# albertz/ParseOggVorbis

Hardware: AMD Instinct MI355X
Metric: audio packets/sec (blocksize 2048, stereo) (higher is better)
Workload: dtype f32; 1 GPU; config3: 65536 stereo packets, blocksize 2048, 64 streams x 1024, floor+coupling+IMDCT+window+overlap-add; packets_per_gpu=65536, parallelism=streams sharded over 1 GPU(s), no data-path collective

## Files before the change

### parseoggvorbis_amd/csrc/vorbis_synth_hip.hip

```cpp
#include <hip/hip_runtime.h>

#include <math.h>
#include <stdarg.h>
#include <stdio.h>
#include <string.h>

#include <algorithm>
#include <cmath>
#include <mutex>
#include <numeric>
#include <string>
#include <vector>

#include <stdlib.h>

#include "vsyn_device.h"
#include "vsyn_staged.h"
#include "vsyn_prep.h"
#include "vsyn_fused.h"
#include "vsyn_fused_u.h"
#include "vsyn_vq.h"
#include "vsyn_pcm.h"
#include "vsyn_features.h"
#include "vsyn_spectral.h"
// ... 224 lines not shown

static int build_const(const vsyn_setup* su, uint32_t max_streams, vsyn_handle* h, const char** err) {
  if (!su) return fail(err, VSYN_ERR_INVALID, "setup is NULL");
  if (su->channels < 1 || su->channels > VSYN_MAX_CHANNELS) return fail(err, VSYN_ERR_INVALID, "channels %u not in 1..%d", su->channels, VSYN_MAX_CHANNELS);
  if (!is_pow2(su->blocksize0) || !is_pow2(su->blocksize1) || su->blocksize0 < VSYN_MIN_BLOCKSIZE ||
      su->blocksize1 > VSYN_MAX_BLOCKSIZE || su->blocksize0 > su->blocksize1)
    return fail(err, VSYN_ERR_INVALID, "blocksizes %u/%u invalid (hpp:1294-1298)", su->blocksize0, su->blocksize1);
  if (su->num_floors < 1 || su->num_floors > VSYN_MAX_TABLES || su->num_mappings < 1 || su->num_mappings > VSYN_MAX_TABLES ||
      su->num_modes < 1 || su->num_modes > VSYN_MAX_TABLES || !su->floors || !su->mappings || !su->modes)
    return fail(err, VSYN_ERR_INVALID, "floor/mapping/mode counts out of range");
  if (max_streams < 1) return fail(err, VSYN_ERR_INVALID, "max_streams must be >= 1");

  ConstHeader& H = h->H;
  memset(&H, 0, sizeof(H));
  H.channels = su->channels;
  H.bs[0] = su->blocksize0;
  H.bs[1] = su->blocksize1;
  H.lg[0] = ilog2(su->blocksize0);
  H.lg[1] = ilog2(su->blocksize1);
  H.num_floors = su->num_floors;
  H.num_mappings = su->num_mappings;
  H.num_modes = su->num_modes;
  H.max_streams = max_streams;

  std::vector<FloorConst> floors(su->num_floors);
  uint32_t maxp = 2;
  for (uint32_t f = 0; f < su->num_floors; ++f) {
    const vsyn_floor1& sf = su->floors[f];
    FloorConst& fc = floors[f];
    memset(&fc, 0, sizeof(fc));
    if (sf.multiplier < 1 || sf.multiplier > 4) return fail(err, VSYN_ERR_INVALID, "floor %u: multiplier %u (hpp:486-492)", f, sf.multiplier);
    if (sf.num_posts < 2 || sf.num_posts > VSYN_MAX_POSTS || !sf.xs) return fail(err, VSYN_ERR_INVALID, "floor %u: %u posts", f, sf.num_posts);
    static const uint32_t range_of[5] = {0, 256, 128, 86, 64};
    fc.mult = sf.multiplier;
    fc.posts = sf.num_posts;
    fc.range = range_of[sf.multiplier];
    maxp = std::max(maxp, sf.num_posts);
    for (uint32_t i = 0; i < sf.num_posts; ++i) {
      if (sf.xs[i] > 0xFFFFu) return fail(err, VSYN_ERR_INVALID, "floor %u: x[%u]=%u too large", f, i, sf.xs[i]);
      fc.xs[i] = (uint16_t)sf.xs[i];
    }
    if (sf.xs[0] != 0) return fail(err, VSYN_ERR_INVALID, "floor %u: xs[0] must be 0 (hpp:449)", f);
    std::vector<uint32_t> order(sf.num_posts);
    for (uint32_t i = 0; i < sf.num_posts; ++i) order[i] = i;
    std::stable_sort(order.begin(), order.end(), [&](uint32_t a, uint32_t b) { return sf.xs[a] < sf.xs[b]; });
    for (uint32_t s = 0; s < sf.num_posts; ++s) {
      if (s && sf.xs[order[s]] == sf.xs[order[s - 1]]) return fail(err, VSYN_ERR_INVALID, "floor %u: duplicate x %u (render_line needs x0<x1, Utils.hpp:145)", f, sf.xs[order[s]]);
      fc.sorted_idx[s] = (uint8_t)order[s];
      fc.xs_sorted[s] = (uint16_t)sf.xs[order[s]];
    }
    for (uint32_t i = 2; i < sf.num_posts; ++i) {
      int lo = -1, hi = -1;
      for (uint32_t j = 0; j < i; ++j) {
        if (sf.xs[j] < sf.xs[i] && (lo < 0 || sf.xs[j] > sf.xs[lo])) lo = (int)j;
        if (sf.xs[j] > sf.xs[i] && (hi < 0 || sf.xs[j] < sf.xs[hi])) hi = (int)j;
      }
      if (lo < 0 || hi < 0) return fail(err, VSYN_ERR_INVALID, "floor %u: post %u has no low/high neighbour (xs[1] must be the maximum)", f, i);
      fc.lo[i] = (uint8_t)lo;
      fc.hi[i] = (uint8_t)hi;
      fc.pk[i].lo = (uint16_t)lo;
      fc.pk[i].hi = (uint16_t)hi;
      fc.pk[i].dxi = (uint16_t)(sf.xs[i] - sf.xs[lo]);
      fc.pk[i].adx = (uint16_t)(sf.xs[hi] - sf.xs[lo]);
      fc.pk[i].inv_adx = 1.0f / (float)(sf.xs[hi] - sf.xs[lo]);
      fc.pk[i].idx = i;
    }
    {
      std::vector<uint32_t> depth(sf.num_posts, 0);
      uint32_t maxd = 0;
      for (uint32_t i = 2; i < sf.num_posts; ++i) {
        depth[i] = 1u + std::max(depth[fc.lo[i]], depth[fc.hi[i]]);
        maxd = std::max(maxd, depth[i]);
      }
      uint32_t ng = 0;
      for (uint32_t d = 1; d <= maxd; ++d) {
        std::vector<uint32_t> at;
        for (uint32_t i = 2; i < sf.num_posts; ++i)
          if (depth[i] == d) at.push_back(i);
        for (size_t k = 0; k < at.size(); k += 4, ++ng)
          for (uint32_t e = 0; e < 4; ++e) fc.sched[ng][e] = fc.pk[at[std::min(k + e, at.size() - 1)]];
      }
      fc.ngroups = ng;
    }
    if (sf.num_posts <= 32)
      for (uint32_t i = 2; i < sf.num_posts; ++i) fc.pk[i].idx = (1u << fc.lo[i]) | (1u << fc.hi[i]) | (1u << i);
  }
  H.ys_stride = (maxp + 3u) & ~3u;
  h->prep_lds_bytes = maxp > 32 ? H.ys_stride * PREP_THREADS * (uint32_t)sizeof(uint32_t) : 16u;
  h->unwrap_lds_bytes = maxp > 32 ? H.ys_stride * UNWRAP_THREADS * (uint32_t)sizeof(uint32_t) : 16u;

  std::vector<MapConst> maps(su->num_mappings);
  for (uint32_t m = 0; m < su->num_mappings; ++m) {
    const vsyn_mapping& sm = su->mappings[m];
    MapConst& mc = maps[m];
    memset(&mc, 0, sizeof(mc));
    if (sm.num_couplings > 256 || (sm.num_couplings && !sm.couplings) || !sm.channel_floor) return fail(err, VSYN_ERR_INVALID, "mapping %u invalid", m);
    mc.ncoup = sm.num_couplings;
    for (uint32_t k = 0; k < sm.num_couplings; ++k) {
      const vsyn_coupling& c = sm.couplings[k];
      if (c.magnitude == c.angle || c.magnitude >= su->channels || c.angle >= su->channels)
        return fail(err, VSYN_ERR_INVALID, "mapping %u coupling %u invalid (hpp:788-790)", m, k);
      mc.coup[2 * k] = c.magnitude;
      mc.coup[2 * k + 1] = c.angle;
    }
    for (uint32_t c = 0; c < su->channels; ++c) {
      if (sm.channel_floor[c] >= su->num_floors) return fail(err, VSYN_ERR_INVALID, "mapping %u: floor index out of range (hpp:807)", m);
      mc.chfloor[c] = sm.channel_floor[c];
    }
  }
  for (uint32_t k = 0; k < su->num_modes; ++k) {
    if (su->modes[k].mapping >= su->num_mappings) return fail(err, VSYN_ERR_INVALID, "mode %u: mapping out of range (hpp:832)", k);
    H.mode_blockflag[k] = su->modes[k].block_flag ? 1 : 0;
    H.mode_mapping[k] = su->modes[k].mapping;
  }

  size_t off = align_up(sizeof(ConstHeader), 256);
  H.off_floor = (uint32_t)off;
  off = align_up(off + sizeof(FloorConst) * floors.size(), 256);
  H.off_map = (uint32_t)off;
  off = align_up(off + sizeof(MapConst) * maps.size(), 256);
  H.off_invdb = (uint32_t)off;
  off = align_up(off + 256 * sizeof(float), 256);
  for (int b = 0; b < 2; ++b) {
    const uint32_t n = H.bs[b];
    H.off_pre[b] = (uint32_t)off;
    off = align_up(off + (n / 4) * sizeof(float2), 256);
    H.off_post[b] = (uint32_t)off;
    off = align_up(off + (n / 4) * sizeof(float2), 256);
    H.off_fft[b] = (uint32_t)off;
    off = align_up(off + (n / 4) * sizeof(float2), 256);
    H.off_win[b] = (uint32_t)off;
    off = align_up(off + 4 * (size_t)n * sizeof(float), 256);
  }
  H.total_bytes = (uint32_t)off;
  h->host_const.assign(off, 0);
  uint8_t* base = h->host_const.data();
  memcpy(base, &H, sizeof(H));
  memcpy(base + H.off_floor, floors.data(), sizeof(FloorConst) * floors.size());
  memcpy(base + H.off_map, maps.data(), sizeof(MapConst) * maps.size());
  memcpy(base + H.off_invdb, k_inverse_db_bits, sizeof(k_inverse_db_bits));
  for (int b = 0; b < 2; ++b) {
    const uint32_t n = H.bs[b], M = n / 2, N4 = n / 4;
    float2* pre = (float2*)(base + H.off_pre[b]);
    float2* post = (float2*)(base + H.off_post[b]);
    float2* tw = (float2*)(base + H.off_fft[b]);
    for (uint32_t k = 0; k < N4; ++k) {
      const double a = -M_PI * (4.0 * k + 1.0) / (4.0 * M);
      pre[k] = make_float2((float)cos(a), (float)sin(a));
      const double p = -M_PI * (double)k / (double)M;
      post[k] = make_float2((float)cos(p), (float)sin(p));
      const double t = -2.0 * M_PI * (double)k / (double)N4;
      tw[k] = make_float2((float)cos(t), (float)sin(t));
    }
    float* win = (float*)(base + H.off_win[b]);
    for (int w = 0; w < 4; ++w) host_window(H.bs[0], H.bs[1], b, w & 1, (w >> 1) & 1, win + (size_t)w * n);
  }
  return VSYN_OK;
}

extern "C" {

const char* vsyn_version(void) { return "parseoggvorbis_amd vsyn 0.1 (gfx950)"; }
int vsyn_abi_version(void) { return VSYN_ABI_VERSION; }

int vsyn_create(const vsyn_setup* setup, int device, uint32_t max_streams, vsyn_handle** out, const char** err) {
  if (!out) return fail(err, VSYN_ERR_INVALID, "out is NULL");
  *out = nullptr;
  int ndev = 0;
// ... 1733 lines not shown
```

### parseoggvorbis_amd/csrc/vsyn_device.h

```cpp
#pragma once
#include <stdint.h>

#include "../../include/vorbis_synth_hip.h"

#define VSYN_SCHED_GROUPS 64
#define VSYN_MAX_TABLES 64

struct FloorConst {
  uint32_t mult, posts, range;
  uint16_t xs[VSYN_MAX_POSTS + 1];
  uint16_t xs_sorted[VSYN_MAX_POSTS + 1];
  uint8_t sorted_idx[VSYN_MAX_POSTS + 3];
  uint8_t lo[VSYN_MAX_POSTS + 3];
  uint8_t hi[VSYN_MAX_POSTS + 3];
  struct PostK {
    uint16_t lo, hi;
    uint16_t dxi, adx;
    float inv_adx;
    uint32_t idx;
  } pk[VSYN_MAX_POSTS + 1];
  uint32_t ngroups, pad_[3];
  PostK sched[VSYN_SCHED_GROUPS][4];
};

struct MapConst {
  uint32_t ncoup;
  uint8_t chfloor[VSYN_MAX_CHANNELS];
  uint16_t coup[2 * 256];
};

struct ConstHeader {
  uint32_t channels, bs[2], lg[2], ys_stride, num_floors, num_mappings, num_modes, max_streams;
  uint32_t off_floor, off_map, off_invdb;
  uint32_t off_pre[2], off_post[2], off_fft[2], off_win[2];
  uint8_t mode_blockflag[VSYN_MAX_TABLES], mode_mapping[VSYN_MAX_TABLES];
  uint32_t total_bytes;
};

struct PktInfo {
  uint64_t res_off;
  uint32_t out_pos;
  uint32_t emit;
  uint32_t used;
  uint32_t own;
  uint16_t n;
  uint8_t lng, widx;
  uint8_t mapping, bad;
  uint16_t pad;
};

struct SegInfo {
  uint32_t has_carry;
  uint32_t carry_n;
  uint32_t parity_in;
  uint32_t total_emit;
};

struct StreamState {
  uint64_t abs_total_pos;
  uint32_t has_prev, prev_n, parity;
  uint32_t tag;
  uint32_t prev_tail;
};

struct DevStatus {
  uint32_t flags, first_bad_packet;
};

#ifdef __HIPCC__
#define VSYN_CPOL_NT 2
typedef float vsyn_nt_f2 __attribute__((ext_vector_type(2)));
typedef float vsyn_nt_f4 __attribute__((ext_vector_type(4)));
__device__ __forceinline__ float2 stream_load2(const float2* p) {
  const vsyn_nt_f2 v = __builtin_nontemporal_load((const vsyn_nt_f2*)p);
  return make_float2(v.x, v.y);
}
__device__ __forceinline__ void stream_store2(float* p, float a, float b) { __builtin_nontemporal_store(vsyn_nt_f2{a, b}, (vsyn_nt_f2*)p); }
__device__ __forceinline__ void stream_store4(float* p, float a, float b, float c, float d) {
  __builtin_nontemporal_store(vsyn_nt_f4{a, b, c, d}, (vsyn_nt_f4*)p);
}
#endif
#ifdef __HIPCC__
__device__ __forceinline__ const ConstHeader* hdr_of(const uint8_t* cb) { return (const ConstHeader*)cb; }
__device__ __forceinline__ const FloorConst* floor_of(const uint8_t* cb, uint32_t f) {
  return (const FloorConst*)(cb + hdr_of(cb)->off_floor) + f;
}
__device__ __forceinline__ const MapConst* map_of(const uint8_t* cb, uint32_t m) {
  return (const MapConst*)(cb + hdr_of(cb)->off_map) + m;
}
__device__ __forceinline__ const float* invdb_of(const uint8_t* cb) { return (const float*)(cb + hdr_of(cb)->off_invdb); }
__device__ __forceinline__ const float2* pre_of(const uint8_t* cb, int b) { return (const float2*)(cb + hdr_of(cb)->off_pre[b]); }
__device__ __forceinline__ const float2* post_of(const uint8_t* cb, int b) { return (const float2*)(cb + hdr_of(cb)->off_post[b]); }
__device__ __forceinline__ const float2* fft_of(const uint8_t* cb, int b) { return (const float2*)(cb + hdr_of(cb)->off_fft[b]); }
__device__ __forceinline__ const float* win_of(const uint8_t* cb, int b, int widx) {
  return (const float*)(cb + hdr_of(cb)->off_win[b]) + (size_t)widx * hdr_of(cb)->bs[b];
}

__device__ __forceinline__ void raise_status(DevStatus* st, uint32_t flag, uint32_t pkt) {
  atomicOr(&st->flags, flag);
  atomicMin(&st->first_bad_packet, pkt);
}

__device__ __forceinline__ StreamState state_read(const StreamState* __restrict__ st, uint32_t stream, uint32_t epoch, uint32_t* slot) {
  const StreamState a = st[2u * stream], b = st[2u * stream + 1u];
  const uint32_t da = (a.tag == 0u || a.tag == epoch) ? 0xFFFFFFFFu : epoch - a.tag;
// ... 43 lines not shown
```

### parseoggvorbis_amd/csrc/vsyn_floor1.h

```cpp
#pragma once
#include <hip/hip_runtime.h>

#include "vsyn_device.h"

typedef __attribute__((address_space(3))) uint32_t floor1_lds_u32;

__device__ __forceinline__ uint32_t render_point_u32(uint32_t x0, uint32_t y0, uint32_t x1, uint32_t y1, uint32_t X) {
  uint32_t adx = x1 - x0;
  bool up = y1 >= y0;
  uint32_t ady = up ? y1 - y0 : y0 - y1;
  uint32_t off = (ady * (X - x0)) / adx;
  return up ? y0 + off : y0 - off;
}

__device__ __forceinline__ void floor1_unwrap_rows(const uint8_t* cb, const uint16_t* ys, uint16_t* fy, DevStatus* status, const bool act,
                                                   const uint32_t fl_id, const uint32_t p, const size_t gid, const uint32_t stride,
                                                   floor1_lds_u32* const col, const uint32_t NT) {
  const FloorConst* const floors = (const FloorConst*)(cb + hdr_of(cb)->off_floor);
  typedef uint32_t u32x16 __attribute__((ext_vector_type(16)));
  typedef const __attribute__((address_space(4))) u32x16* const_grp;
  typedef const __attribute__((address_space(4))) uint32_t* kptr;
  uint64_t todo = __ballot(act);
  while (todo) {
    const uint32_t f = __builtin_amdgcn_readlane(fl_id, (uint32_t)__builtin_ctzll(todo));
    const bool mine = act && fl_id == f;
    todo &= ~__ballot(mine);
    const FloorConst* fc = floors + f;
    const uint32_t posts = *(kptr)(uintptr_t)&fc->posts, range = *(kptr)(uintptr_t)&fc->range, mult = *(kptr)(uintptr_t)&fc->mult;
    const uint32_t ngroups = *(kptr)(uintptr_t)&fc->ngroups;
    if (!mine) continue;
    if (posts <= 32u) {
      uint32_t fr[32];
      const uint2* in8 = (const uint2*)(ys + gid * stride);
      uint2 win[8];
#pragma unroll
      for (uint32_t j = 0; j < 8; ++j) {
        win[j] = make_uint2(0u, 0u);
        if (j * 4 < posts) win[j] = in8[j];
      }
      uint32_t flags = 3;
      bool bad = false;
      typedef const __attribute__((address_space(4))) u32x16* const_pk4;
      for (int attempt = 0; attempt < 2; ++attempt) {
        const bool exact = attempt == 1;
#pragma unroll
        for (uint32_t j = 0; j < 8; ++j) {
          fr[4 * j + 0] = win[j].x & 0xFFFFu;
          fr[4 * j + 1] = win[j].x >> 16;
          fr[4 * j + 2] = win[j].y & 0xFFFFu;
          fr[4 * j + 3] = win[j].y >> 16;
        }
        flags = 3;
        bad = false;
        uint32_t big_acc = 0;
        auto step = [&](const uint32_t i, const uint32_t kx, const uint32_t ky, const uint32_t kz, const uint32_t touched) {
          const uint32_t lo = kx & 0xFFFFu, hi = kx >> 16;
          const uint32_t val = fr[i], ylo = fr[lo], yhi = fr[hi];
          const uint32_t dxi = ky & 0xFFFFu, adx = ky >> 16;
          const bool up = yhi >= ylo;
          const uint32_t ady = up ? yhi - ylo : ylo - yhi;
          const uint32_t prod = ady * dxi;
          uint32_t off;
          if (exact) {
            off = prod / adx;
          } else {
            off = (uint32_t)(((float)prod + 0.5f) * __uint_as_float(kz));
            big_acc |= prod >> 21;
          }
          const uint32_t predicted = up ? ylo + off : ylo - off;
          const bool ok = predicted <= range;
          const uint32_t pr = ok ? predicted : 0u;
          const uint32_t high_room = range - pr;
          const uint32_t m = min(high_room, pr);
          const uint32_t d = val - m;
          const uint32_t dbig = high_room > pr ? d : ~d;
          const uint32_t dsmall = (val >> 1) ^ (0u - (val & 1u));
          const uint32_t delta = val >= 2u * m ? dbig : dsmall;
          const uint32_t fn = val == 0 ? pr : pr + delta;
          flags |= val != 0 ? touched : 0u;
          bad = bad || !ok;
          fr[i] = bad ? 0u : fn;
        };
        u32x16 kn = *(const_pk4)(uintptr_t)&fc->pk[2];
        for (uint32_t i = 2; i < posts; i += 4) {
          const u32x16 kq = kn;
          kn = *(const_pk4)(uintptr_t)&fc->pk[i + 4];
          step(i, kq[0], kq[1], kq[2], kq[3]);
          if (i + 1 < posts) step(i + 1, kq[4], kq[5], kq[6], kq[7]);
          if (i + 2 < posts) step(i + 2, kq[8], kq[9], kq[10], kq[11]);
          if (i + 3 < posts) step(i + 3, kq[12], kq[13], kq[14], kq[15]);
        }
        if (exact || !__any(big_acc != 0u)) break;
        if (big_acc == 0u) break;
      }
      uint2* out8 = (uint2*)(fy + gid * stride);
      if (bad) raise_status(status, VSYN_ST_FLOOR_RANGE, p);
#pragma unroll
      for (uint32_t j = 0; j < 8; ++j) {
        if (j * 4 >= posts) break;
        uint32_t w[4];
#pragma unroll
        for (uint32_t e = 0; e < 4; ++e) {
          const uint32_t i = 4 * j + e;
          uint32_t v = fr[i] * mult;
          if (v > 0x7FFFu || fr[i] > 0x7FFFu) v = 0x7FFFu;
          w[e] = i < posts ? (bad ? 0x8000u : (v | (((flags >> i) & 1u) << 15))) : 0u;
        }
        out8[j] = make_uint2(w[0] | (w[1] << 16), w[2] | (w[3] << 16));
      }
      continue;
    }
    {
      const uint2* in8 = (const uint2*)(ys + gid * stride);
      for (uint32_t j = 0; j * 4 < posts; ++j) {
        const uint2 w = in8[j];
        col[(4 * j + 0) * NT] = w.x & 0xFFFFu;
        col[(4 * j + 1) * NT] = w.x >> 16;
        col[(4 * j + 2) * NT] = w.y & 0xFFFFu;
        col[(4 * j + 3) * NT] = w.y >> 16;
      }
    }
    uint64_t flags_lo = 3;
    uint32_t flag_64 = 0;
    bool bad = false;
    u32x16 kn = *(const_grp)(uintptr_t)&fc->sched[0][0];
    for (uint32_t gi = 0; gi < ngroups; ++gi) {
      const u32x16 kq = kn;
      kn = *(const_grp)(uintptr_t)&fc->sched[gi + 1u < VSYN_SCHED_GROUPS ? gi + 1u : gi][0];
      uint32_t val[4], ylo[4], yhi[4], fn[4], prod[4], off[4];
#pragma unroll
      for (int e = 0; e < 4; ++e) {
        val[e] = col[kq[4 * e + 3] * NT];
        ylo[e] = col[(kq[4 * e] & 0xFFFFu) * NT];
        yhi[e] = col[(kq[4 * e] >> 16) * NT];
      }
      bool any_big = false;
#pragma unroll
      for (int e = 0; e < 4; ++e) {
        const uint32_t dxi = kq[4 * e + 1] & 0xFFFFu;
        const bool up = yhi[e] >= ylo[e];
        const uint32_t ady = up ? yhi[e] - ylo[e] : ylo[e] - yhi[e];
        prod[e] = ady * dxi;
        off[e] = (uint32_t)(((float)prod[e] + 0.5f) * __uint_as_float(kq[4 * e + 2]));
        any_big = any_big || prod[e] >= (1u << 21) || ady >= 65536u;
      }
      if (__any(any_big)) {
#pragma unroll
        for (int e = 0; e < 4; ++e) {
          const bool up = yhi[e] >= ylo[e];
          const uint32_t ady = up ? yhi[e] - ylo[e] : ylo[e] - yhi[e];
          if (prod[e] >= (1u << 21) || ady >= 65536u) off[e] = prod[e] / (kq[4 * e + 1] >> 16);
        }
      }
#pragma unroll
      for (int e = 0; e < 4; ++e) {
        const bool up = yhi[e] >= ylo[e];
        const uint32_t predicted = up ? ylo[e] + off[e] : ylo[e] - off[e];
        const bool ok = predicted <= range;
        const uint32_t pr = ok ? predicted : 0u;
        const uint32_t high_room = range - pr, low_room = pr;
        const uint32_t room = min(high_room, low_room) * 2;
        const uint32_t big = high_room > low_room ? val[e] - low_room + pr : pr - val[e] + high_room - 1;
        const uint32_t small = (val[e] & 1u) ? pr - (val[e] + 1) / 2 : pr + val[e] / 2;
        fn[e] = val[e] == 0 ? pr : (val[e] >= room ? big : small);
        const uint32_t lo = kq[4 * e] & 0xFFFFu, hi = kq[4 * e] >> 16, i = kq[4 * e + 3];
        const uint64_t touched = (1ull << lo) | (1ull << hi) | (i < 64u ? 1ull << i : 0ull);
        flags_lo |= val[e] != 0 ? touched : 0ull;
        flag_64 |= (val[e] != 0 && i >= 64u) ? 1u : 0u;
        bad = bad || !ok;
      }
#pragma unroll
      for (int e = 0; e < 4; ++e) col[kq[4 * e + 3] * NT] = bad ? 0u : fn[e];
    }
    uint2* out8 = (uint2*)(fy + gid * stride);
    if (bad) raise_status(status, VSYN_ST_FLOOR_RANGE, p);
    for (uint32_t j = 0; j * 4 < posts; ++j) {
      uint32_t w[4];
#pragma unroll
      for (uint32_t e = 0; e < 4; ++e) {
        const uint32_t i = 4 * j + e;
        const uint32_t fv = i < posts ? col[i * NT] : 0u;
        uint32_t v = fv * mult;
        if (v > 0x7FFFu || fv > 0x7FFFu) v = 0x7FFFu;
        const uint32_t fl = i < 64 ? (uint32_t)((flags_lo >> i) & 1ull) : (i == 64 ? flag_64 : 0u);
        w[e] = i < posts ? (bad ? 0x8000u : (v | (fl << 15))) : 0u;
      }
      out8[j] = make_uint2(w[0] | (w[1] << 16), w[2] | (w[3] << 16));
    }
  }
}

// ... 13 lines not shown
```

### parseoggvorbis_amd/csrc/vsyn_prep.h

```cpp
#pragma once
#include <hip/hip_runtime.h>

#include "vsyn_device.h"
#include "vsyn_floor1.h"
#include "vsyn_staged.h"

#define PREP_MAX_SEG_PACKETS 4096u
#define PREP_WAVES 4
#define PREP_THREADS (PREP_WAVES * 64)

struct PrepCtx {
  const uint8_t* cb;
  const vsyn_packet* packets;
  const vsyn_segment* segs;
  const uint16_t* ys;
  uint16_t* fy;
  PktInfo* info;
  SegInfo* sinfo;
  StreamState* state;
  DevStatus* status;
  uint32_t* emit_len;
  uint8_t* run_cls;
  uint64_t plane_stride, long_modes;
  uint32_t S, R, runs_per_seg, fused_ok, P, epoch;
// ... 49 lines not shown
    const uint64_t r = s_res[w];
    if (w < wv) {
      pre = abs_combine(pre, a);
      rpre += r;
    }
    tot = abs_combine(tot, a);
    rtot += r;
  }
  inc = abs_combine(pre, inc);
  rinc += rpre;
  *total = tot;
  *rtotal = rtot;
}

__global__ void __launch_bounds__(PREP_THREADS) vsyn_prep_kernel(const PrepCtx A) {
  extern __shared__ __attribute__((aligned(16))) uint32_t s_rows[];
  __shared__ AbsScan s_abs[PREP_WAVES];
  __shared__ uint64_t s_res[PREP_WAVES];
  __shared__ uint32_t s_pk[PREP_THREADS];
  __shared__ uint32_t s_longbits[PREP_MAX_SEG_PACKETS / 32 + 2];
  __shared__ uint32_t s_last_n;
  const uint8_t* __restrict__ cb = A.cb;
  const ConstHeader* H = hdr_of(cb);
  const uint32_t t = threadIdx.x, lane = t & 63u, wave = __builtin_amdgcn_readfirstlane(t >> 6);
  const uint32_t NT = blockDim.x;
  const uint32_t C = H->channels;
  const uint32_t xj = blockIdx.x >> 3;
  const uint32_t role = (xj ^ (xj >> 5)) & 1u, bid = ((xj >> 1) << 3) | (blockIdx.x & 7u);
  const uint32_t g = bid / A.chunks_per_seg, ch = bid % A.chunks_per_seg;
  if (g >= A.S) return;
#ifdef PREP_STAMPS
  unsigned long long pst_acc[PREP_NSTAMPS] = {0, 0, 0, 0, 0, 0, 0, 0};
  unsigned long long pst_last = __builtin_readcyclecounter();
  const unsigned long long pst_t0 = __builtin_amdgcn_s_memrealtime();
#define PSTAMP_FLUSH()                                                                                              \
  do {                                                                                                              \
    const uint32_t unit_ = blockIdx.x * PREP_WAVES + wave;                                                          \
    if (lane == 0 && unit_ < 8192) {                                                                                \
      for (int i_ = 0; i_ < 5; ++i_) g_prep_stamps[unit_][i_] = pst_acc[i_];                                        \
      g_prep_stamps[unit_][5] = pst_t0;                                                                             \
      g_prep_stamps[unit_][6] = __builtin_amdgcn_s_memrealtime();                                                   \
      g_prep_stamps[unit_][7] = 1ull + role;                                                                        \
    }                                                                                                               \
  } while (0)
#else
#define PSTAMP_FLUSH() do { } while (0)
#endif
  const vsyn_segment sg = A.segs[g];
  const uint32_t num = sg.num_packets;
  const uint32_t R = A.R;
  const uint32_t run0 = ch * A.chunk_runs;
  const uint32_t run1 = min(A.runs_per_seg, run0 + A.chunk_runs);
  const uint32_t cs = run0 * R;
  uint8_t* const cls_row = A.run_cls + (size_t)g * A.runs_per_seg;
  if (sg.stream >= H->max_streams || (uint64_t)sg.first_packet + sg.num_packets > A.P || (sg.residue_off & 3)) {
    if (role) return;
    for (uint32_t r = run0 + t; r < run1; r += NT) cls_row[r] = 0xFFu;
    if (ch == 0u && t == 0u) {
      raise_status(A.status, VSYN_ST_BAD_SEGMENT, sg.first_packet < A.P ? sg.first_packet : 0);
      A.sinfo[g] = SegInfo{0, 0, 0, 0};
    }
    return;
  }
  const uint32_t ce = min(num, run1 * R);
  const vsyn_packet* const spk = A.packets + sg.first_packet;
  typedef uint32_t u32x4 __attribute__((ext_vector_type(4)));
  const uint32_t num_modes = H->num_modes, bs0 = H->bs[0], bs1 = H->bs[1];
  const uint64_t long_modes = A.long_modes;
#define PREP_IS_LONG(m) ((m) < num_modes && (m) < 64u && ((long_modes >> (m)) & 1ull))
#define PREP_N_OF_MODE(m) (PREP_IS_LONG(m) ? bs1 : bs0)
  if (role) {
    const uint32_t ce = min(num, run1 * R);
    if (cs >= ce) return;
    const vsyn_packet* const spk = A.packets + sg.first_packet;
    const uint32_t stride = __builtin_amdgcn_readfirstlane(H->ys_stride);
    const MapConst* const maps = (const MapConst*)(cb + H->off_map);
    const uint32_t chan_mask = C >= 32 ? 0xFFFFFFFFu : ((1u << C) - 1u);
    const uint32_t num_modes = H->num_modes;
    const uint32_t ppp = NT / C;
    for (uint32_t base = cs; base < ce; base += ppp) {
      const uint32_t pe = min(ce, base + ppp);
      const uint32_t rp = t / C, c = t - rp * C;
      const bool row_ok = rp < pe - base;
      uint32_t kmode = 0xFFFFFFFFu, fused_mask = 0;
      if (row_ok) {
        typedef uint32_t u32x2 __attribute__((ext_vector_type(2)));
        const u32x2 w = *(const u32x2*)(spk + base + rp);
        kmode = w.x & 0xFFu;
        fused_mask = w.y;
      }
      const bool mode_ok = row_ok && kmode < num_modes;
      uint32_t fl_id = 0xFFFFFFFFu;
      {
        typedef const __attribute__((address_space(4))) uint32_t* kptr;
        uint64_t todo = __ballot(mode_ok);
        while (todo) {
          const uint32_t m = __builtin_amdgcn_readlane(kmode, (uint32_t)__builtin_ctzll(todo));
          const bool mine = mode_ok && kmode == m;
          todo &= ~__ballot(mine);
          const uint32_t mw = *(kptr)(uintptr_t)((const uint8_t*)H->mode_mapping + (m & ~3u));
          const uint32_t mp = (mw >> (8u * (m & 3u))) & 0xFFu;
          if (mine) fl_id = maps[mp].chfloor[c];
        }
      }
      const bool act = mode_ok && (((fused_mask & chan_mask) >> c) & 1u);
      const uint32_t prow = sg.first_packet + base + rp;
      PSTAMP(3);
      floor1_unwrap_rows(A.cb, A.ys, A.fy, A.status, act, fl_id, prow, (size_t)prow * C + c, stride, (floor1_lds_u32*)s_rows + t, NT);
      PSTAMP(4);
    }
    PSTAMP_FLUSH();
    return;
  }
  uint32_t st_slot;
  const StreamState st0 = state_read(A.state, sg.stream, A.epoch, &st_slot);
  const bool reset = (sg.flags & VSYN_SEG_RESET) != 0;
  const uint32_t carry_n = (!reset && st0.has_prev) ? st0.prev_n : 0;
  const int64_t abs0 = reset ? 0 : (int64_t)st0.abs_total_pos;
  SegInfo si;
  si.has_carry = carry_n ? 1u : 0u;
  si.carry_n = carry_n;
  si.parity_in = reset ? 0u : st0.parity;
  si.total_emit = 0;
  if (cs >= num) {
    for (uint32_t r = run0 + t; r < run1; r += NT) cls_row[r] = 0xFFu;
    if (num == 0u && ch == 0u && t == 0u) {
      A.sinfo[g] = si;
      if (reset) state_write(A.state, sg.stream, st_slot, StreamState{0, 0, 0, 0, 0}, A.epoch);
    }
    return;
  }
  PSTAMP(0);

  AbsScan cin = {0, 0};
  uint64_t cres = 0;
  uint32_t prev_n_in = carry_n;
  uint32_t prev_tail_in = carry_n ? st0.prev_tail : 0u;
  bool halo_long = !carry_n;
  if (cs > 0u) {
    const uint32_t per = (cs + NT - 1u) / NT;
    const uint32_t b = min(cs, t * per), e = min(cs, b + per);
    AbsScan agg = {0, 0};
    uint64_t res = 0;
    uint32_t prev_n = 0;
    if (b < e) prev_n = b == 0u ? carry_n : PREP_N_OF_MODE((uint32_t)spk[b - 1u].mode);
    constexpr uint32_t KEEP = 8;
    for (uint32_t base = b; base < e; base += KEEP) {
      u32x4 kq[KEEP];
#pragma unroll
      for (uint32_t j = 0; j < KEEP; ++j)
        if (base + j < e) kq[j] = *(const u32x4*)(spk + base + j);
#pragma unroll
      for (uint32_t j = 0; j < KEEP; ++j)
        if (base + j < e) {
          const uint32_t md = kq[j].x & 0xFFu;
          const uint32_t n = PREP_N_OF_MODE(md);
          const int64_t gran = (int64_t)((uint64_t)kq[j].z | ((uint64_t)kq[j].w << 32));
          agg = abs_combine(agg, abs_element(gran, prev_n ? (int64_t)(prev_n / 4 + n / 4) : 0));
          res += (uint64_t)C * (n / 2);
          prev_n = n;
        }
    }
    prep_block_scan(agg, res, s_abs, s_res, &cin, &cres);
    const uint32_t hm = __builtin_amdgcn_readfirstlane((uint32_t)spk[cs - 1u].mode);
    prev_n_in = PREP_N_OF_MODE(hm);
    halo_long = PREP_IS_LONG(hm);
    prev_tail_in = prev_tail_of(PREP_IS_LONG(hm), (uint8_t)__builtin_amdgcn_readfirstlane((uint32_t)spk[cs - 1u].next_long));
  }
  PSTAMP(1);

  const uint32_t stride = __builtin_amdgcn_readfirstlane(H->ys_stride);
  const MapConst* const maps = (const MapConst*)(cb + H->off_map);
  const uint32_t chan_mask = C >= 32 ? 0xFFFFFFFFu : ((1u << C) - 1u);
  const uint32_t ppp = NT / C;
  for (uint32_t w = t; w < (ce - cs + 1u + 31u) / 32u; w += NT) s_longbits[w] = 0u;
  __syncthreads();
  if (t == 0u && halo_long) s_longbits[0] = 1u;
  for (uint32_t base = cs; base < ce; base += ppp) {
    const uint32_t pe = min(ce, base + ppp);
    const uint32_t q = base + t;
    const bool valid = q < pe;
    vsyn_packet k = {};
    if (valid) {
      const u32x4 w = *(const u32x4*)(spk + q);
      k.mode = (uint8_t)(w.x & 0xFFu);
      k.prev_long = (uint8_t)((w.x >> 8) & 0xFFu);
      k.next_long = (uint8_t)((w.x >> 16) & 0xFFu);
      k.floor_used = w.y;
      k.granule = (int64_t)((uint64_t)w.z | ((uint64_t)w.w << 32));
    }
    const bool mode_ok = valid && k.mode < num_modes;
// ... 116 lines not shown
```

### parseoggvorbis_amd/csrc/vsyn_staged.h

```cpp
#pragma once
#include <hip/hip_runtime.h>

#include "vsyn_device.h"
#include "vsyn_floor1.h"

struct AbsScan {
  int64_t val;
  int set;
  int64_t lo;
};
__device__ __forceinline__ AbsScan abs_combine(AbsScan a, AbsScan b) {
  AbsScan r;
  r.val = a.val + b.val;
  r.set = a.set | b.set;
  r.lo = b.set ? (a.set ? max(b.lo, a.lo + b.val) : b.lo) : a.lo + b.val;
  return r;
}
__device__ __forceinline__ AbsScan abs_element(int64_t granule, int64_t L) {
  AbsScan e;
  e.set = granule >= 0;
  e.val = e.set ? 0 : L;
  e.lo = e.set ? granule : 0;
  return e;
}
// ... 347 lines not shown
                                  plane_stride, C);
      if (ps.raise & VSYN_ST_BAD_MODE) raise_status(status, VSYN_ST_BAD_MODE, p);
      if (ps.raise & VSYN_ST_WINDOW_FLAGS) raise_status(status, VSYN_ST_WINDOW_FLAGS, p);
      if (ps.raise & VSYN_ST_GRANULE) raise_status(status, VSYN_ST_GRANULE, p);
      if (ps.raise & VSYN_ST_PLANE_OVERFLOW) raise_status(status, VSYN_ST_PLANE_OVERFLOW, p);
      info[p] = ps.pi;
      if (mode_ok && lng) atomicOr(&s_longbits[(ql + 1u) >> 5], 1u << ((ql + 1u) & 31u));
      seg_of_pkt[p] = g;
      if (emit_len) emit_len[p] = ps.pi.emit;
      if (q == num - 1) {
        s_abs_end = ps.abs_after;
        s_last_n = n;
        s_last_tail = prev_tail_of(mode_ok && lng, k.next_long);
      }
      abs_before = ps.abs_after;
      res_off += (uint64_t)C * (n / 2);
      prev_n = n;
      prev_tail = prev_tail_of(mode_ok && lng, k.next_long);
    };
    for (uint32_t base = qb; base < qe; base += KEEP) {
      if (!keep) {
#pragma unroll
        for (uint32_t j = 0; j < KEEP; ++j)
          if (base + j < qe) kq[j] = spk[cs + base + j];
      }
#pragma unroll
      for (uint32_t j = 0; j < KEEP; ++j)
        if (base + j < qe) step_b(base + j, kq[j]);
    }
  }
  __syncthreads();

  {
    const uint32_t nruns = (num + R - 1) / R;
    for (uint32_t r = ch * runs_per_chunk + t; r < min(runs_per_seg, (ch + 1u) * runs_per_chunk); r += NT) {
      const uint32_t qa = r * R, qb2 = min(num, qa + R);
      const uint32_t cls = r >= nruns ? 0xFFu
                                      : run_class_bits(s_longbits, qa - cs + 1u, qb2 - cs + 1u, qa == 0 ? carry_n : 0u, fused_ok, qa == 0);
      run_cls[(size_t)g * runs_per_seg + r] = (uint8_t)cls;
      if (r >= nruns || cls) continue;
      const bool prev_fast = qa > 0 && run_class(H, spk, qa - R, qa, carry_n, fused_ok) != 0;
      const uint32_t cnt = (qb2 - qa) + (prev_fast ? 1u : 0u);
      uint32_t at = atomicAdd(staged_count, cnt);
      if (prev_fast) staged_list[at++] = sg.first_packet + qa - 1;
      for (uint32_t q = qa; q < qb2; ++q) staged_list[at++] = (sg.first_packet + q) | 0x80000000u;
    }
  }
  if (t == 0 && (last_chunk || num == 0)) {
    SegInfo si;
    si.has_carry = carry_n ? 1u : 0u;
    si.carry_n = carry_n;
    si.parity_in = reset ? 0u : st0.parity;
    if (num == 0) {
      si.total_emit = 0;
      sinfo[g] = si;
      if (reset) state_write(state, sg.stream, st_slot, StreamState{0, 0, 0, 0, 0}, epoch);
      return;
    }
    si.total_emit = (uint32_t)(s_abs_end - abs0);
    sinfo[g] = si;
    StreamState ns;
    ns.abs_total_pos = (uint64_t)s_abs_end;
    ns.has_prev = 1;
    ns.prev_n = s_last_n;
    ns.prev_tail = s_last_tail;
    ns.parity = si.parity_in ^ 1u;
    ns.tag = 0;
    state_write(state, sg.stream, st_slot, ns, epoch);
  }
}

#define UNWRAP_THREADS 128
__global__ void __launch_bounds__(UNWRAP_THREADS)
vsyn_floor_unwrap_kernel(const uint8_t* __restrict__ cb, uint32_t P, const PktInfo* __restrict__ info, const uint16_t* __restrict__ ys,
                         uint16_t* __restrict__ fy_out, DevStatus* __restrict__ status) {
  extern __shared__ __attribute__((aligned(16))) uint32_t s_rows[];
  const ConstHeader* H = hdr_of(cb);
  const uint32_t C = H->channels, stride = __builtin_amdgcn_readfirstlane(H->ys_stride), t = threadIdx.x;
  const uint32_t rows = P * C;
  for (uint32_t base = blockIdx.x * UNWRAP_THREADS; base < rows; base += gridDim.x * UNWRAP_THREADS) {
    const uint32_t row = base + t, p = row / C, c = row - p * C;
    bool act = false;
    uint32_t fl_id = 0xFFFFFFFFu;
    if (row < rows) {
      const PktInfo pi = info[p];
      act = !pi.bad && ((pi.own >> c) & 1u);
      if (act) fl_id = map_of(cb, pi.mapping)->chfloor[c];
    }
    floor1_unwrap_rows(cb, ys, fy_out, status, act, fl_id, p, row, stride, (floor1_lds_u32*)s_rows + t, UNWRAP_THREADS);
  }
}

__device__ __forceinline__ void inverse_couple(float& m, float& a) {
  const float d = m > 0.f ? a : -a;
  const float x = m - d, y = m + d;
  const bool ap = a > 0.f;
  a = ap ? x : m;
  m = ap ? m : y;
}

__global__ void __launch_bounds__(256)
vsyn_spectrum_kernel(const uint8_t* __restrict__ cb, const uint32_t* __restrict__ list, const uint32_t* __restrict__ count,
                     const PktInfo* __restrict__ info, const float* __restrict__ residue, const uint16_t* __restrict__ fy,
                     float* __restrict__ env, uint16_t* __restrict__ curve_tap, DevStatus* __restrict__ status) {
  const ConstHeader* H = hdr_of(cb);
  const uint32_t total = *count;
  for (uint32_t li = blockIdx.x; li < total; li += gridDim.x) {
  const uint32_t p = list[li] & 0x7FFFFFFFu;
  const PktInfo pi = info[p];
  if (pi.bad) continue;
  const uint32_t n2 = pi.n / 2u, C = H->channels;
  for (uint32_t i = threadIdx.x; i < n2; i += 256) {
  const float* src = residue + pi.res_off;
  float* dst = env + pi.res_off;
  for (uint32_t c = 0; c < C; ++c) dst[(size_t)c * n2 + i] = src[(size_t)c * n2 + i];
  const MapConst* mc = map_of(cb, pi.mapping);
  for (uint32_t k = mc->ncoup; k > 0; --k) {
    const uint32_t m = mc->coup[2 * (k - 1)], a = mc->coup[2 * (k - 1) + 1];
    float mv = dst[(size_t)m * n2 + i], av = dst[(size_t)a * n2 + i];
    inverse_couple(mv, av);
    dst[(size_t)m * n2 + i] = mv;
    dst[(size_t)a * n2 + i] = av;
  }
  const float* invdb = invdb_of(cb);
  for (uint32_t c = 0; c < C; ++c) {
    if (!((pi.used >> c) & 1u)) continue;
    float f = 0.f;
    if ((pi.own >> c) & 1u) {
      const FloorConst* fc = floor_of(cb, mc->chfloor[c]);
      const uint32_t v = floor1_curve_at(fc, fy + ((size_t)p * C + c) * H->ys_stride, i);
      if (curve_tap) curve_tap[pi.res_off + (size_t)c * n2 + i] = (uint16_t)min(v, 65535u);
      if (v >= 256u) {
        raise_status(status, VSYN_ST_FLOOR_VALUE, p);
        f = 0.f;
      } else {
        f = invdb[v];
      }
    }
    dst[(size_t)c * n2 + i] *= f;
  }
  }
  }
}

__device__ __forceinline__ float2 cmul(float2 a, float2 b) {
  return make_float2(__builtin_fmaf(a.x, b.x, -(a.y * b.y)), __builtin_fmaf(a.x, b.y, a.y * b.x));
}

__device__ void imdct_block_lds(const uint8_t* __restrict__ cb, int b, uint32_t n, const float* __restrict__ X,
                                float* __restrict__ y, float2* bufA, float2* bufB) {
  const uint32_t M = n / 2, N4 = n / 4, T = blockDim.x, t = threadIdx.x;
  const float2* pre = pre_of(cb, b);
  const float2* post = post_of(cb, b);
  const float2* tw = fft_of(cb, b);
  for (uint32_t k = t; k < N4; k += T) bufA[k] = cmul(make_float2(X[2 * k], X[M - 1 - 2 * k]), pre[k]);
  __syncthreads();
  float2* src = bufA;
  float2* dst = bufB;
  for (uint32_t Ns = 1; Ns < N4; Ns <<= 1) {
    const uint32_t tstride = N4 / (2 * Ns);
    for (uint32_t j = t; j < N4 / 2; j += T) {
      const uint32_t k = j & (Ns - 1);
      const float2 v0 = src[j];
      const float2 v1 = cmul(src[j + N4 / 2], tw[k * tstride]);
      const uint32_t o = ((j - k) << 1) + k;
      dst[o] = make_float2(v0.x + v1.x, v0.y + v1.y);
      dst[o + Ns] = make_float2(v0.x - v1.x, v0.y - v1.y);
    }
    __syncthreads();
    float2* tmp = src;
    src = dst;
    dst = tmp;
// ... 100 lines not shown
```

Measured before the change: 270.9 million packets/s.

## Prefetch floor rows early and unroll floor1 unwrap with register-resident post table

```diff
diff --git a/parseoggvorbis_amd/csrc/vorbis_synth_hip.hip b/parseoggvorbis_amd/csrc/vorbis_synth_hip.hip
--- a/parseoggvorbis_amd/csrc/vorbis_synth_hip.hip
+++ b/parseoggvorbis_amd/csrc/vorbis_synth_hip.hip
@@ -330,8 +330,19 @@
       }
       fc.ngroups = ng;
     }
-    if (sf.num_posts <= 32)
-      for (uint32_t i = 2; i < sf.num_posts; ++i) fc.pk[i].idx = (1u << fc.lo[i]) | (1u << fc.hi[i]) | (1u << i);
+    if (sf.num_posts <= 32) {
+      memset(fc.sched, 0, sizeof(fc.sched));
+      for (uint32_t i = 2; i < sf.num_posts; ++i) {
+        FloorConst::PostR& r = fc.reg[i];
+        r.lo = fc.lo[i];
+        r.hi = fc.hi[i];
+        r.fdxi = (float)fc.pk[i].dxi;
+        r.inv_adx = fc.pk[i].inv_adx;
+        r.touched = (1u << fc.lo[i]) | (1u << fc.hi[i]) | (1u << i);
+        r.dxi = fc.pk[i].dxi;
+        r.adx = fc.pk[i].adx;
+      }
+    }
   }
   H.ys_stride = (maxp + 3u) & ~3u;
   h->prep_lds_bytes = maxp > 32 ? H.ys_stride * PREP_THREADS * (uint32_t)sizeof(uint32_t) : 16u;
diff --git a/parseoggvorbis_amd/csrc/vsyn_device.h b/parseoggvorbis_amd/csrc/vsyn_device.h
--- a/parseoggvorbis_amd/csrc/vsyn_device.h
+++ b/parseoggvorbis_amd/csrc/vsyn_device.h
@@ -20,7 +20,16 @@
     uint32_t idx;
   } pk[VSYN_MAX_POSTS + 1];
   uint32_t ngroups, pad_[3];
-  PostK sched[VSYN_SCHED_GROUPS][4];
+  struct PostR {
+    uint32_t lo, hi;
+    float fdxi, inv_adx;
+    uint32_t touched;
+    uint32_t dxi, adx, pad_;
+  };
+  union {
+    PostK sched[VSYN_SCHED_GROUPS][4];
+    PostR reg[34];
+  };
 };
 
 struct MapConst {
diff --git a/parseoggvorbis_amd/csrc/vsyn_floor1.h b/parseoggvorbis_amd/csrc/vsyn_floor1.h
--- a/parseoggvorbis_amd/csrc/vsyn_floor1.h
+++ b/parseoggvorbis_amd/csrc/vsyn_floor1.h
@@ -13,9 +13,53 @@
   return up ? y0 + off : y0 - off;
 }
 
+__device__ __forceinline__ void floor1_load_row(const uint16_t* ys, const bool ok, const size_t gid, const uint32_t stride, uint2 (&win)[8]) {
+  const uint2* in8 = (const uint2*)(ys + gid * stride);
+#pragma unroll
+  for (uint32_t j = 0; j < 8; ++j) {
+    win[j] = make_uint2(0u, 0u);
+    if (ok && j * 4 < stride) win[j] = in8[j];
+  }
+}
+
+typedef uint32_t floor1_u32x8 __attribute__((ext_vector_type(8)));
+typedef uint32_t floor1_u32x16 __attribute__((ext_vector_type(16)));
+
+template <uint32_t I>
+__device__ __forceinline__ void floor1_chain_post(uint32_t (&fr)[32], const floor1_u32x8 k, const uint32_t range, uint32_t& flags, uint32_t& worst,
+                                                  uint32_t& big) {
+  const uint32_t val = fr[I], ylo = fr[k[0]], yhi = fr[k[1]];
+  uint32_t ady;
+  asm("v_sad_u32 %0, %1, %2, 0" : "=v"(ady) : "v"(yhi), "v"(ylo));
+  const float prod = (float)ady * __uint_as_float(k[2]);
+  big = max(big, __float_as_uint(prod));
+  const uint32_t off = (uint32_t)((prod + 0.5f) * __uint_as_float(k[3]));
+  const uint32_t pr = yhi >= ylo ? ylo + off : ylo - off;
+  worst = max(worst, pr);
+  const uint32_t high_room = range - pr, m = min(high_room, pr), half = val >> 1;
+  const uint32_t fsmall = (half ^ (0u - (val & 1u))) + pr;
+  const uint32_t fbig = high_room > pr ? val : range - 1u - val;
+  const uint32_t fn = half >= m ? fbig : fsmall;
+  flags |= val != 0 ? k[4] : 0u;
+  fr[I] = val == 0 ? pr : fn;
+}
+
+template <uint32_t I>
+__device__ __forceinline__ void floor1_chain(uint32_t (&fr)[32], const FloorConst* fc, const uint32_t posts, const uint32_t range, uint32_t& flags,
+                                             uint32_t& worst, uint32_t& big, const floor1_u32x16 kq) {
+  if constexpr (I < 32) {
+    typedef const __attribute__((address_space(4))) floor1_u32x16* const_reg2;
+    if (I >= posts) return;
+    const floor1_u32x16 kn = *(const_reg2)(uintptr_t)&fc->reg[I + 2];
+    floor1_chain_post<I>(fr, floor1_u32x8{kq[0], kq[1], kq[2], kq[3], kq[4], kq[5], kq[6], kq[7]}, range, flags, worst, big);
+    if (I + 1 < posts) floor1_chain_post<I + 1>(fr, floor1_u32x8{kq[8], kq[9], kq[10], kq[11], kq[12], kq[13], kq[14], kq[15]}, range, flags, worst, big);
+    floor1_chain<I + 2>(fr, fc, posts, range, flags, worst, big, kn);
+  }
+}
+
 __device__ __forceinline__ void floor1_unwrap_rows(const uint8_t* cb, const uint16_t* ys, uint16_t* fy, DevStatus* status, const bool act,
                                                    const uint32_t fl_id, const uint32_t p, const size_t gid, const uint32_t stride,
-                                                   floor1_lds_u32* const col, const uint32_t NT) {
+                                                   floor1_lds_u32* const col, const uint32_t NT, const uint2 (&win)[8]) {
   const FloorConst* const floors = (const FloorConst*)(cb + hdr_of(cb)->off_floor);
   typedef uint32_t u32x16 __attribute__((ext_vector_type(16)));
   typedef const __attribute__((address_space(4))) u32x16* const_grp;
@@ -30,19 +74,20 @@
     const uint32_t ngroups = *(kptr)(uintptr_t)&fc->ngroups;
     if (!mine) continue;
     if (posts <= 32u) {
+      typedef const __attribute__((address_space(4))) floor1_u32x8* const_reg;
+      typedef const __attribute__((address_space(4))) floor1_u32x16* const_reg2;
       uint32_t fr[32];
-      const uint2* in8 = (const uint2*)(ys + gid * stride);
-      uint2 win[8];
 #pragma unroll
       for (uint32_t j = 0; j < 8; ++j) {
-        win[j] = make_uint2(0u, 0u);
-        if (j * 4 < posts) win[j] = in8[j];
-      }
-      uint32_t flags = 3;
-      bool bad = false;
-      typedef const __attribute__((address_space(4))) u32x16* const_pk4;
-      for (int attempt = 0; attempt < 2; ++attempt) {
-        const bool exact = attempt == 1;
+        fr[4 * j + 0] = win[j].x & 0xFFFFu;
+        fr[4 * j + 1] = win[j].x >> 16;
+        fr[4 * j + 2] = win[j].y & 0xFFFFu;
+        fr[4 * j + 3] = win[j].y >> 16;
+      }
+      uint32_t flags = 3, worst = 0, big = 0;
+      floor1_chain<2>(fr, fc, posts, range, flags, worst, big, *(const_reg2)(uintptr_t)&fc->reg[2]);
+      bool bad = worst > range;
+      if (big >= 0x4A000000u) {
 #pragma unroll
         for (uint32_t j = 0; j < 8; ++j) {
           fr[4 * j + 0] = win[j].x & 0xFFFFu;
@@ -52,21 +97,12 @@
         }
         flags = 3;
         bad = false;
-        uint32_t big_acc = 0;
-        auto step = [&](const uint32_t i, const uint32_t kx, const uint32_t ky, const uint32_t kz, const uint32_t touched) {
-          const uint32_t lo = kx & 0xFFFFu, hi = kx >> 16;
-          const uint32_t val = fr[i], ylo = fr[lo], yhi = fr[hi];
-          const uint32_t dxi = ky & 0xFFFFu, adx = ky >> 16;
+        for (uint32_t i = 2; i < posts; ++i) {
+          const floor1_u32x8 k = *(const_reg)(uintptr_t)&fc->reg[i];
+          const uint32_t val = fr[i], ylo = fr[k[0]], yhi = fr[k[1]];
           const bool up = yhi >= ylo;
           const uint32_t ady = up ? yhi - ylo : ylo - yhi;
-          const uint32_t prod = ady * dxi;
-          uint32_t off;
-          if (exact) {
-            off = prod / adx;
-          } else {
-            off = (uint32_t)(((float)prod + 0.5f) * __uint_as_float(kz));
-            big_acc |= prod >> 21;
-          }
+          const uint32_t off = (ady * k[5]) / k[6];
           const uint32_t predicted = up ? ylo + off : ylo - off;
           const bool ok = predicted <= range;
           const uint32_t pr = ok ? predicted : 0u;
@@ -77,21 +113,10 @@
           const uint32_t dsmall = (val >> 1) ^ (0u - (val & 1u));
           const uint32_t delta = val >= 2u * m ? dbig : dsmall;
           const uint32_t fn = val == 0 ? pr : pr + delta;
-          flags |= val != 0 ? touched : 0u;
+          flags |= val != 0 ? k[4] : 0u;
           bad = bad || !ok;
           fr[i] = bad ? 0u : fn;
-        };
-        u32x16 kn = *(const_pk4)(uintptr_t)&fc->pk[2];
-        for (uint32_t i = 2; i < posts; i += 4) {
-          const u32x16 kq = kn;
-          kn = *(const_pk4)(uintptr_t)&fc->pk[i + 4];
-          step(i, kq[0], kq[1], kq[2], kq[3]);
-          if (i + 1 < posts) step(i + 1, kq[4], kq[5], kq[6], kq[7]);
-          if (i + 2 < posts) step(i + 2, kq[8], kq[9], kq[10], kq[11]);
-          if (i + 3 < posts) step(i + 3, kq[12], kq[13], kq[14], kq[15]);
-        }
-        if (exact || !__any(big_acc != 0u)) break;
-        if (big_acc == 0u) break;
+        }
       }
       uint2* out8 = (uint2*)(fy + gid * stride);
       if (bad) raise_status(status, VSYN_ST_FLOOR_RANGE, p);
@@ -102,11 +127,11 @@
 #pragma unroll
         for (uint32_t e = 0; e < 4; ++e) {
           const uint32_t i = 4 * j + e;
-          uint32_t v = fr[i] * mult;
-          if (v > 0x7FFFu || fr[i] > 0x7FFFu) v = 0x7FFFu;
-          w[e] = i < posts ? (bad ? 0x8000u : (v | (((flags >> i) & 1u) << 15))) : 0u;
-        }
-        out8[j] = make_uint2(w[0] | (w[1] << 16), w[2] | (w[3] << 16));
+          const uint32_t v = min(min(fr[i], 0x7FFFu) * mult, 0x7FFFu);
+          w[e] = v | (((flags >> i) & 1u) << 15);
+        }
+        const uint32_t k0 = (4 * j + 1 < posts ? 0xFFFF0000u : 0u) | 0xFFFFu, k1 = (4 * j + 2 < posts ? 0xFFFFu : 0u) | (4 * j + 3 < posts ? 0xFFFF0000u : 0u);
+        out8[j] = make_uint2((bad ? 0x80008000u : (w[0] | (w[1] << 16))) & k0, (bad ? 0x80008000u : (w[2] | (w[3] << 16))) & k1);
       }
       continue;
     }
diff --git a/parseoggvorbis_amd/csrc/vsyn_prep.h b/parseoggvorbis_amd/csrc/vsyn_prep.h
--- a/parseoggvorbis_amd/csrc/vsyn_prep.h
+++ b/parseoggvorbis_amd/csrc/vsyn_prep.h
@@ -155,6 +155,9 @@
       const uint32_t pe = min(ce, base + ppp);
       const uint32_t rp = t / C, c = t - rp * C;
       const bool row_ok = rp < pe - base;
+      const uint32_t prow = sg.first_packet + base + rp;
+      uint2 win[8];
+      floor1_load_row(A.ys, row_ok, (size_t)prow * C + c, stride, win);
       uint32_t kmode = 0xFFFFFFFFu, fused_mask = 0;
       if (row_ok) {
         typedef uint32_t u32x2 __attribute__((ext_vector_type(2)));
@@ -177,9 +180,8 @@
         }
       }
       const bool act = mode_ok && (((fused_mask & chan_mask) >> c) & 1u);
-      const uint32_t prow = sg.first_packet + base + rp;
       PSTAMP(3);
-      floor1_unwrap_rows(A.cb, A.ys, A.fy, A.status, act, fl_id, prow, (size_t)prow * C + c, stride, (floor1_lds_u32*)s_rows + t, NT);
+      floor1_unwrap_rows(A.cb, A.ys, A.fy, A.status, act, fl_id, prow, (size_t)prow * C + c, stride, (floor1_lds_u32*)s_rows + t, NT, win);
       PSTAMP(4);
     }
     PSTAMP_FLUSH();
diff --git a/parseoggvorbis_amd/csrc/vsyn_staged.h b/parseoggvorbis_amd/csrc/vsyn_staged.h
--- a/parseoggvorbis_amd/csrc/vsyn_staged.h
+++ b/parseoggvorbis_amd/csrc/vsyn_staged.h
@@ -453,12 +453,14 @@
     const uint32_t row = base + t, p = row / C, c = row - p * C;
     bool act = false;
     uint32_t fl_id = 0xFFFFFFFFu;
+    uint2 win[8];
+    floor1_load_row(ys, row < rows, row, stride, win);
     if (row < rows) {
       const PktInfo pi = info[p];
       act = !pi.bad && ((pi.own >> c) & 1u);
       if (act) fl_id = map_of(cb, pi.mapping)->chfloor[c];
     }
-    floor1_unwrap_rows(cb, ys, fy_out, status, act, fl_id, p, row, stride, (floor1_lds_u32*)s_rows + t, UNWRAP_THREADS);
+    floor1_unwrap_rows(cb, ys, fy_out, status, act, fl_id, p, row, stride, (floor1_lds_u32*)s_rows + t, UNWRAP_THREADS, win);
   }
 }
 
```

Result: no change. 270.5 million packets/s, median of 2 (-0.1%).
